# lipku/LiveTalking

Measured on NVIDIA H100. Metric: lip-sync frames/sec (wav2lip256, 256x256, batch 16, mel + U-Net fwd + paste-back), higher is better.
Workload: dtype f16 (fp32 accumulate); mel f64; paste u8

## Files before the change

livetalking_b200/csrc/conv_halo.cu:

```cuda
#include <cuda.h>

#include <atomic>
#include <mutex>
#include <utility>

#include "conv_halo.h"
#include "ltb_internal.h"
#include "ptx_sm90.cuh"

#ifdef LTB_HALO_DIAG
#include <cstdlib>
#define LTB_DIAG(bit) (p.dbg & (bit))
#else
#define LTB_DIAG(bit) 0
#endif

namespace ltb {

constexpr int kHaloP = 10;
constexpr int kHaloThreads = 384;
constexpr int kProducerRegs = 40, kConsumerRegs = 232;
constexpr int kSms = 132;

template <int BN, int NSUB, int NACC, int TAPS, int RC = 0>
struct HaloCfg {
  static constexpr bool HALO = (TAPS != 1);
  static constexpr bool S2 = (TAPS == 10);
  static constexpr int P = S2 ? 9 : (HALO ? kHaloP : 8);
  static constexpr int HR = S2 ? 16 * NSUB + 1 : (HALO ? 16 * NSUB + 2 : 16 * NSUB);
  static constexpr int TG = (TAPS == 9 || TAPS == 10) ? 3 : (TAPS == 16 ? 4 : 1);
  static constexpr int PLANE_BYTES = (HR * P * 128 + 1023) & ~1023;
  static constexpr int A_BYTES_RAW = (S2 ? 4 : 1) * HR * P * 128;
  static constexpr int A_BYTES = S2 ? 4 * PLANE_BYTES : ((A_BYTES_RAW + 1023) & ~1023);
  static constexpr int B_BYTES = TG * BN * 128;
  static constexpr int BUDGET = 223 * 1024;
  static constexpr int A_STAGES_STREAM = S2 ? 2 : ((BN <= 32) ? 4 : (BN <= 64 ? 3 : (NSUB == 1 ? 3 : 2)));
  static constexpr int A_STAGES_RES = ((BUDGET - RC * TG * B_BYTES) / A_BYTES) > 4 ? 4 : ((BUDGET - RC * TG * B_BYTES) / A_BYTES);
  static constexpr int A_STAGES = RC ? A_STAGES_RES : A_STAGES_STREAM;
  static constexpr int B_STAGES_MAX = (BUDGET - A_STAGES * A_BYTES) / B_BYTES;
  static constexpr int B_STAGES = RC ? RC * TG : (B_STAGES_MAX > 8 ? 8 : B_STAGES_MAX);
  static constexpr bool LAG = RC || B_STAGES >= 2 * TG;
  static constexpr int ACOLS = NACC * BN;
  static constexpr int SMEM_BYTES = A_STAGES * A_BYTES + B_STAGES * B_BYTES + 1024;
  static_assert(NSUB * ACOLS <= 256, "register accumulator overflow");
  static_assert(B_STAGES >= 2, "not enough shared memory for the weight ring");
  static_assert(A_STAGES >= 2, "not enough shared memory for the halo ring");
  static_assert(SMEM_BYTES + 3584 <= 227 * 1024, "shared memory overflow (dynamic + static)");
};

struct SubpixelView {
  int stage, view, slot0, brow, nslots;
};
constexpr int subpixel_view(int vy, int vx) { return (vy + 1) * kHaloP + (vx + 1); }
template <int TAPS>
struct SubpixelTable;
template <>
struct SubpixelTable<9> {
  static constexpr int NV = 5;
  static constexpr SubpixelView v[NV] = {{0, 0, 0, 0, 3}, {1, 1, 1, 0, 2}, {1, kHaloP + 1, 2, 2, 1}, {2, 0, 3, 2, 1}, {2, kHaloP, 2, 0, 2}};
};
template <>
struct SubpixelTable<16> {
  static constexpr int NV = 10;
  static constexpr SubpixelView v[NV] = {{0, subpixel_view(0, 0), 0, 0, 4},
                                         {1, subpixel_view(-1, 0), 0, 0, 2},  {1, subpixel_view(0, 1), 1, 2, 2},
                                         {2, subpixel_view(1, 0), 2, 0, 2},   {2, subpixel_view(0, -1), 0, 2, 1}, {2, subpixel_view(0, -1), 3, 3, 1},
                                         {3, subpixel_view(-1, -1), 0, 0, 1}, {3, subpixel_view(-1, 1), 1, 1, 1}, {3, subpixel_view(1, 1), 2, 2, 1},
                                         {3, subpixel_view(1, -1), 3, 3, 1}};
};

template <int BN, int SLOT0, int BROW, int R, size_t... S>
__device__ __forceinline__ void subpixel_slots(float (&acc)[R], uint64_t a, uint32_t b_lo, uint32_t b_hi, std::index_sequence<S...>) {
  (wgmma_ss_at<BN, (SLOT0 + (int)S) * BN>(acc, a, wgmma_lohi(b_lo + (BROW + (uint32_t)S) * BN * 8u, b_hi), 1u), ...);
}

template <int BN, int TAPS, int R, size_t... V>
__device__ __forceinline__ void subpixel_issue(float (&acc)[R], int j, int k, uint32_t a_lo0, uint32_t b_lo0, uint32_t a_hi, uint32_t b_hi,
                                               std::index_sequence<V...>) {
  (
      [&] {
        constexpr SubpixelView g = SubpixelTable<TAPS>::v[V];
        if (j == g.stage)
          subpixel_slots<BN, g.slot0, g.brow>(acc, wgmma_lohi(a_lo0 + g.view * 8u + k * 2u, a_hi), b_lo0 + k * 2u, b_hi,
                                              std::make_index_sequence<g.nslots>{});
      }(),
      ...);
}

__device__ __forceinline__ void quad_transpose(uint32_t (&x)[4], int lane) {
  const bool b2 = lane & 2, b1 = lane & 1;
  uint32_t s0 = __shfl_xor_sync(0xffffffffu, b2 ? x[0] : x[2], 2);
  uint32_t s1 = __shfl_xor_sync(0xffffffffu, b2 ? x[1] : x[3], 2);
  x[0] = b2 ? s0 : x[0];
  x[1] = b2 ? s1 : x[1];
  x[2] = b2 ? x[2] : s0;
  x[3] = b2 ? x[3] : s1;
  s0 = __shfl_xor_sync(0xffffffffu, b1 ? x[0] : x[1], 1);
  s1 = __shfl_xor_sync(0xffffffffu, b1 ? x[2] : x[3], 1);
  x[0] = b1 ? s0 : x[0];
  x[2] = b1 ? s1 : x[2];
  x[1] = b1 ? x[1] : s0;
  x[3] = b1 ? x[3] : s1;
}

constexpr bool halo_res_smem_ok(int BN, int NSUB, int NACC, int TAPS) { return TAPS == 9 && NACC == 1 && BN * NSUB <= 128; }

template <int BN, int NSUB, int NACC, int TAPS, int RC, bool GRP>
__global__ void __launch_bounds__(kHaloThreads, 1) conv_halo_wgmma_kernel(const __grid_constant__ HaloParams p) {
  static_assert(!GRP || TAPS == 1, "grouped weights exist in GEMM mode only");
  using C = HaloCfg<BN, NSUB, NACC, TAPS, RC>;
  extern __shared__ uint8_t smem_raw[];
  __shared__ __align__(8) uint64_t a_full[C::A_STAGES], a_empty[C::A_STAGES];
  __shared__ __align__(8) uint64_t b_full[C::B_STAGES], b_empty[C::B_STAGES];
  __shared__ float head_sw[100];
  constexpr int kGnSmem = (NACC == 1) ? 512 : 1;
  __shared__ float gn_acc[kGnSmem];

  const int tid = threadIdx.x, warp = tid >> 5, lane = tid & 31;
  constexpr bool kHeadOk = (BN == 32 && NACC == 1 && TAPS == 9);
  const bool gn_smem = NACC == 1 && p.gn_stats != nullptr && p.gn_images * p.gn_groups * 2 <= kGnSmem;
  if (gn_smem)
    for (int i = tid; i < p.gn_images * p.gn_groups * 2; i += kHaloThreads) gn_acc[i] = 0.f;
  constexpr bool kHaloMode = C::HALO;
  if (kHeadOk && p.head_out && tid < 99) head_sw[tid] = (tid < 96) ? p.head_w[tid] : p.head_b[tid - 96];
  const uint32_t smem0 = (smem_u32(smem_raw) + 1023u) & ~1023u;
  const uint32_t a_smem = smem0;
  const uint32_t b_smem = smem0 + C::A_STAGES * C::A_BYTES;
  const int chunks = (p.Cin + 63) / 64;

  if (tid == 0) {
    for (int s = 0; s < C::A_STAGES; ++s) {
      mbar_init(smem_u32(&a_full[s]), 1);
      mbar_init(smem_u32(&a_empty[s]), 8);
    }
    for (int s = 0; s < C::B_STAGES; ++s) {
      mbar_init(smem_u32(&b_full[s]), 1);
      mbar_init(smem_u32(&b_empty[s]), 8);
    }
    mbar_fence_init();
    tma_prefetch_desc(&p.tm_in);
    tma_prefetch_desc(&p.tm_w);
  }
  __syncthreads();

  const int tiles_m = kHaloMode ? p.tiles_x * p.tiles_y * p.N : p.tiles_x;

  pdl_launch_dependents();
  if (RC && warp == 8 && lane == 0) {
    mbar_arrive_expect_tx(smem_u32(&b_full[0]), RC * C::TG * C::B_BYTES);
    for (int c = 0; c < RC; ++c)
      for (int j = 0; j < C::TG; ++j)
        tma_load_3d(b_smem + (c * C::TG + j) * C::B_BYTES, &p.tm_w, smem_u32(&b_full[0]), c * 64, 0, j * C::TG);
  }
  pdl_wait();

  if (warp >= 8) {
    setmaxnreg_dec<kProducerRegs>();
    if (warp == 8 && lane == 0) {
      uint32_t ai = 0, bi = 0;
      for (int t = blockIdx.x; t < p.total_tiles; t += gridDim.x) {
        const int nt = t / tiles_m;
        int mt = t - nt * tiles_m;
        int img = 0, y0 = 0, x0 = 0;
        int g_row = 0, g_slot = 0;
        if constexpr (GRP) {
          const int g = mt / p.group_tiles;
          g_row = g * p.group_rows + (mt - g * p.group_tiles) * (128 * NSUB);
          g_slot = p.group_slot[g];
        }
        if (kHaloMode) {
          img = mt / (p.tiles_x * p.tiles_y);
          mt -= img * (p.tiles_x * p.tiles_y);
          const int ty = mt / p.tiles_x, tx = mt - ty * p.tiles_x;
          y0 = ty * (16 * NSUB) + p.halo_y0;
          x0 = tx * 8 + p.halo_x0;
        }
        for (int c = 0; c < chunks; ++c) {
          const uint32_t as = ai % C::A_STAGES;
          mbar_wait(smem_u32(&a_empty[as]), ((ai / C::A_STAGES) & 1u) ^ 1u);
          if (LTB_DIAG(8)) {
            mbar_arrive(smem_u32(&a_full[as]));
          } else {
            mbar_arrive_expect_tx(smem_u32(&a_full[as]), C::A_BYTES_RAW);
            if (C::S2) {
#pragma unroll
              for (int pl = 0; pl < 4; ++pl)
                tma_load_4d(a_smem + as * C::A_BYTES + pl * C::PLANE_BYTES, &p.tm_in, smem_u32(&a_full[as]), c * 64,
                            2 * (x0 + 1) - (pl & 1), 2 * (y0 + 1) - (pl >> 1), img);
            } else if (kHaloMode) tma_load_4d(a_smem + as * C::A_BYTES, &p.tm_in, smem_u32(&a_full[as]), c * 64, x0, y0, img);
            else if constexpr (GRP) tma_load_2d(a_smem + as * C::A_BYTES, &p.tm_in, smem_u32(&a_full[as]), c * 64, g_row);
            else tma_load_2d(a_smem + as * C::A_BYTES, &p.tm_in, smem_u32(&a_full[as]), c * 64, mt * (128 * NSUB));
          }
          ++ai;
          if (RC) continue;
          for (int j = 0; j < C::TG; ++j) {
            const uint32_t bs = bi % C::B_STAGES;
            mbar_wait(smem_u32(&b_empty[bs]), ((bi / C::B_STAGES) & 1u) ^ 1u);
            if (LTB_DIAG(16)) {
              mbar_arrive(smem_u32(&b_full[bs]));
              ++bi;
              continue;
            }
            mbar_arrive_expect_tx(smem_u32(&b_full[bs]), C::B_BYTES);
            if (kHaloMode) tma_load_3d(b_smem + bs * C::B_BYTES, &p.tm_w, smem_u32(&b_full[bs]), c * 64, nt * BN, j * C::TG);
            else if constexpr (GRP) tma_load_3d(b_smem + bs * C::B_BYTES, &p.tm_w, smem_u32(&b_full[bs]), c * 64, nt * BN, g_slot);
            else tma_load_2d(b_smem + bs * C::B_BYTES, &p.tm_w, smem_u32(&b_full[bs]), c * 64, nt * BN);
            ++bi;
          }
        }
      }
    }
  } else {
    setmaxnreg_inc<kConsumerRegs>();
    const int wg = warp >> 2, wq = warp & 3;
    const int cq = 2 * (lane & 3);
    constexpr uint32_t kAHi = wgmma_hi_128b(C::P * 128);
    constexpr uint32_t kBHi = wgmma_hi_128b(1024);
    constexpr uint32_t kRowsPerSub = C::HALO ? 16u * C::P : 128u;
    const uint32_t wg_off = (uint32_t)wg * (C::HALO ? 8u * C::P : 64u) * 8u;
    constexpr bool kResHalo = halo_res_smem_ok(BN, NSUB, NACC, TAPS);
    const int res_row = (8 * wg + 2 * wq + ((lane >> 3) & 1) + 1) * C::P + (lane & 7) + 1;
    const int res_kb = lane >> 4;
    if (RC) mbar_wait(smem_u32(&b_full[0]), 0);
    uint32_t ai = 0, bi = 0;
    for (int t = blockIdx.x; t < p.total_tiles; t += gridDim.x) {
      float acc[NSUB][C::ACOLS / 2];
#pragma unroll
      for (int s = 0; s < NSUB; ++s)
#pragma unroll
        for (int i = 0; i < C::ACOLS / 2; ++i) acc[s][i] = 0.f;
      uint32_t rh[NSUB][2][BN / 8];
      const int n0_res = (t / tiles_m) * BN;
      const int c_res = (kResHalo && p.res_halo) ? n0_res / 64 : chunks;
      const int cb_res = (BN == 32) ? (n0_res & 63) >> 3 : 0;
      uint32_t pend_as = 0, pend_bs = 0;
      bool pend = false;
#pragma unroll 1
      for (int c = 0; c < chunks; ++c) {
        const uint32_t as = ai % C::A_STAGES;
        mbar_wait(smem_u32(&a_full[as]), (ai / C::A_STAGES) & 1u);
        if constexpr (kResHalo) {
          if (c == c_res || (BN == 128 && c == c_res + 1)) {
            const bool hi = BN == 128 && c != c_res;
            const uint32_t rbase = a_smem + as * C::A_BYTES + res_row * 128;
#pragma unroll
            for (int s = 0; s < NSUB; ++s)
#pragma unroll
              for (int i = 0; i < BN / 8; i += 2) {
                if (BN == 128 && (i >= 8) != hi) continue;
                const uint32_t chunk16 = (uint32_t)(((cb_res + i + res_kb) & 7) ^ (res_row & 7));
                ldmatrix_x4(rh[s][0][i], rh[s][1][i], rh[s][0][i + 1], rh[s][1][i + 1], rbase + s * (16 * C::P * 128) + chunk16 * 16);
              }
          }
        }
        const uint32_t a_lo0 = wgmma_lo(a_smem + as * C::A_BYTES) + wg_off;
        const uint32_t bs0 = bi % C::B_STAGES;
#pragma unroll
        for (int j = 0; j < C::TG; ++j) {
          const uint32_t bs = RC ? (uint32_t)(c * C::TG + j) : (bi + j) % C::B_STAGES;
          if (!RC) mbar_wait(smem_u32(&b_full[bs]), ((bi + j) / C::B_STAGES) & 1u);
          const uint32_t b_lo0 = wgmma_lo(b_smem + bs * C::B_BYTES);
          if (!LTB_DIAG(4)) wgmma_fence();
#pragma unroll
          for (int k = 0; k < 4; ++k) {
            if (LTB_DIAG(4)) break;
            if constexpr (NACC == 1) {
#pragma unroll
              for (int tt = 0; tt < C::TG; ++tt) {
                const uint32_t aoff = C::S2 ? (uint32_t)(((j != 1) * 2 + (tt != 1)) * (C::PLANE_BYTES / 16) + ((j == 2) * C::P + (tt == 2)) * 8)
                                            : (kHaloMode ? (uint32_t)(j * C::P + tt) * 8u : 0u);
                const uint64_t bd = wgmma_lohi(b_lo0 + tt * (BN * 8) + k * 2, kBHi);
#pragma unroll
                for (int sub = 0; sub < NSUB; ++sub)
                  Wgmma<BN>::ss(acc[sub], wgmma_lohi(a_lo0 + aoff + sub * kRowsPerSub * 8 + k * 2, kAHi), bd, 1u);
              }
            } else {
              subpixel_issue<BN, TAPS>(acc[0], j, k, a_lo0, b_lo0, kAHi, kBHi, std::make_index_sequence<SubpixelTable<TAPS>::NV>{});
            }
          }
          if constexpr (!C::LAG) {
            wgmma_commit();
            wgmma_wait<0>();
            __syncwarp();
            if (lane == 0) mbar_arrive(smem_u32(&b_empty[bs]));
          }
        }
        if (C::LAG) {
          wgmma_commit();
          wgmma_wait<1>();
          if (pend) {
            __syncwarp();
            if (lane == 0) {
              mbar_arrive(smem_u32(&a_empty[pend_as]));
              if (!RC)
                for (int j = 0; j < C::TG; ++j) mbar_arrive(smem_u32(&b_empty[(pend_bs + j) % C::B_STAGES]));
            }
          }
          pend = true;
          pend_as = as;
          pend_bs = bs0;
        } else {
          __syncwarp();
          if (lane == 0) mbar_arrive(smem_u32(&a_empty[as]));
        }
        ++ai;
        if (!RC) bi += C::TG;
      }
      wgmma_wait<0>();
#pragma unroll
      for (int s = 0; s < NSUB; ++s) wgmma_fence_regs(acc[s]);
      if (C::LAG && pend) {
        __syncwarp();
        if (lane == 0) {
          mbar_arrive(smem_u32(&a_empty[pend_as]));
          if (!RC)
            for (int j = 0; j < C::TG; ++j) mbar_arrive(smem_u32(&b_empty[(pend_bs + j) % C::B_STAGES]));
        }
      }
      if (LTB_DIAG(2)) continue;

      const int nt = t / tiles_m;
      int mt = t - nt * tiles_m;
      int img = 0, ty = 0, tx = 0;
      if (kHaloMode) {
        img = mt / (p.tiles_x * p.tiles_y);
        mt -= img * (p.tiles_x * p.tiles_y);
        ty = mt / p.tiles_x;
        tx = mt - ty * p.tiles_x;
      }
      const int n0 = nt * BN;
      const float* bias = p.bias;
      int g_tile = 0;
      if constexpr (GRP) {
        g_tile = mt / p.group_tiles;
        bias += p.group_slot[g_tile] * p.bias_slot_stride;
      }
      const bool has_res = (p.res != nullptr) && !LTB_DIAG(1);
      const bool res_smem = kResHalo && has_res && p.res_halo;
      const bool res_gmem = has_res && !res_smem;
      const bool head = kHeadOk && p.head_out != nullptr;
      float2 bb[BN / 8];
#pragma unroll
      for (int i = 0; i < BN / 8; ++i) bb[i] = __ldg(reinterpret_cast<const float2*>(bias + n0 + 8 * i + cq));
      const __half2 hmax = __floats2half2_rn(65504.f, 65504.f);
      const __half2 hlo = p.relu ? __floats2half2_rn(0.f, 0.f) : __floats2half2_rn(-65504.f, -65504.f);
      auto add_res = [&](uint32_t v, uint32_t r) {
        const __half2 o = __hmin2(__hmax2(__hadd2(*reinterpret_cast<const __half2*>(&v), *reinterpret_cast<const __half2*>(&r)), hlo), hmax);
        return *reinterpret_cast<const uint32_t*>(&o);
      };
#pragma unroll
      for (int sub = 0; sub < NSUB; ++sub) {
        float gs[BN / 8], gq[BN / 8];
#pragma unroll
        for (int i = 0; i < BN / 8; ++i) gs[i] = gq[i] = 0.f;
#pragma unroll
        for (int sl = 0; sl < NACC; ++sl) {
#pragma unroll
          for (int hh = 0; hh < 2; ++hh) {
            const int r = wq * 16 + (lane >> 2) + 8 * hh;
            size_t opix;
            bool row_ok;
            if (kHaloMode) {
              const int gy = ty * (16 * NSUB) + sub * 16 + wg * 8 + (r >> 3), gx = tx * 8 + (r & 7);
              opix = ((size_t)img * p.OH + gy * p.osy + p.acc_oy[sl]) * p.OW + gx * p.osx + p.acc_ox[sl];
              row_ok = gy < p.GH && gx < p.GW;
            } else if constexpr (GRP) {
              const int lrow = (mt - g_tile * p.group_tiles) * (128 * NSUB) + sub * 128 + wg * 64 + r;
              opix = (size_t)g_tile * p.group_rows + lrow;
              row_ok = lrow < p.group_rows;
            } else {
              opix = (size_t)mt * (128 * NSUB) + sub * 128 + wg * 64 + r;
              row_ok = opix < (size_t)p.M;
            }
            const size_t ocol = n0 + 8 * (lane & 3);
            uint4* optr = reinterpret_cast<uint4*>(p.out + opix * p.OCtot + p.oc_off + ocol);
            const uint4* rptr = res_gmem ? reinterpret_cast<const uint4*>(p.res + opix * p.RCtot + p.rc_off + ocol) : nullptr;
            __half2 oh[BN / 8];
#pragma unroll
            for (int m = 0; m < BN / 32; ++m) {
              uint32_t v[4];
#pragma unroll
              for (int j = 0; j < 4; ++j) {
                const int i = 4 * m + j;
                const float f0 = acc[sub][sl * BN / 2 + 4 * i + 2 * hh] + bb[i].x;
                const float f1 = acc[sub][sl * BN / 2 + 4 * i + 2 * hh + 1] + bb[i].y;
                v[j] = (!has_res && p.relu) ? f32x2_to_f16x2_sat_relu(f0, f1) : f32x2_to_f16x2_sat(f0, f1);
                if constexpr (kResHalo)
                  if (res_smem) v[j] = add_res(v[j], rh[sub][hh][i]);
                oh[i] = *reinterpret_cast<const __half2*>(&v[j]);
              }
              if (!head || res_gmem) {
                quad_transpose(v, lane);
                if (res_gmem) {
                  uint4 r4 = make_uint4(0u, 0u, 0u, 0u);
                  if (row_ok) r4 = __ldcg(rptr + 4 * m);
                  const uint32_t rv[4] = {r4.x, r4.y, r4.z, r4.w};
#pragma unroll
                  for (int j = 0; j < 4; ++j) v[j] = add_res(v[j], rv[j]);
                }
                if (row_ok && !head && !LTB_DIAG(1)) optr[4 * m] = make_uint4(v[0], v[1], v[2], v[3]);
                if (res_gmem && (p.gn_stats || head)) {
                  quad_transpose(v, lane);
#pragma unroll
                  for (int j = 0; j < 4; ++j) oh[4 * m + j] = *reinterpret_cast<const __half2*>(&v[j]);
                }
              }
            }
            if (p.gn_stats && row_ok) {
#pragma unroll
              for (int i = 0; i < BN / 8; ++i) {
                const float2 f = __half22float2(oh[i]);
                gs[i] += f.x + f.y;
                gq[i] += f.x * f.x + f.y * f.y;
              }
            }
            if constexpr (kHeadOk) {
              if (head) {
                uint32_t hv[4][4];
#pragma unroll
                for (int src = 0; src < 4; ++src)
#pragma unroll
                  for (int i = 0; i < 4; ++i)
                    hv[src][i] = __shfl_sync(0xffffffffu, *reinterpret_cast<uint32_t*>(&oh[i]), (lane & ~3) + src);
                if ((lane & 3) == 0 && row_ok) {
                  float ha0 = head_sw[96], ha1 = head_sw[97], ha2 = head_sw[98];
#pragma unroll
                  for (int i = 0; i < 4; ++i)
#pragma unroll
                    for (int src = 0; src < 4; ++src) {
                      const float2 f = __half22float2(*reinterpret_cast<__half2*>(&hv[src][i]));
                      const int cc = 8 * i + 2 * src;
                      ha0 = fmaf(f.x, head_sw[cc], ha0);
                      ha0 = fmaf(f.y, head_sw[cc + 1], ha0);
                      ha1 = fmaf(f.x, head_sw[32 + cc], ha1);
                      ha1 = fmaf(f.y, head_sw[32 + cc + 1], ha1);
                      ha2 = fmaf(f.x, head_sw[64 + cc], ha2);
                      ha2 = fmaf(f.y, head_sw[64 + cc + 1], ha2);
                    }
                  float* o = p.head_out + opix * 3;
                  o[0] = (1.f / (1.f + expf(-ha0))) * 255.f;
                  o[1] = (1.f / (1.f + expf(-ha1))) * 255.f;
                  o[2] = (1.f / (1.f + expf(-ha2))) * 255.f;
                }
              }
            }
          }
        }
        const size_t gn_row0 = (size_t)mt * (128 * NSUB) + sub * 128 + wg * 64 + wq * 16;
        if (p.gn_stats && (kHaloMode || gn_row0 < (size_t)p.M)) {
          int gimg = img;
          if (!kHaloMode) gimg = (int)(gn_row0 / (size_t)p.gn_hw);
          float* sbase = (gn_smem ? gn_acc : p.gn_stats) + (size_t)gimg * p.gn_groups * 2;
#pragma unroll
          for (int i = 0; i < BN / 8; ++i) {
            float a = gs[i], b = gq[i];
#pragma unroll
            for (int o = 4; o < 32; o <<= 1) {
              a += __shfl_xor_sync(0xffffffffu, a, o);
              b += __shfl_xor_sync(0xffffffffu, b, o);
            }
            a += __shfl_xor_sync(0xffffffffu, a, 1);
            b += __shfl_xor_sync(0xffffffffu, b, 1);
            if (p.gn_cpg >= 8) {
              a += __shfl_xor_sync(0xffffffffu, a, 2);
              b += __shfl_xor_sync(0xffffffffu, b, 2);
            }
            if (lane == 0 || (p.gn_cpg == 4 && lane == 2)) {
              const int g = (n0 + 8 * i + cq) / p.gn_cpg;
              atomicAdd(sbase + 2 * g, a);
              atomicAdd(sbase + 2 * g + 1, b);
            }
          }
        }
      }
    }
  }

  __syncthreads();
  if (gn_smem) {
    for (int i = tid; i < p.gn_images * p.gn_groups * 2; i += kHaloThreads) {
      const float v = gn_acc[i];
      if (v != 0.f) atomicAdd(p.gn_stats + i, v);
    }
  }
}

typedef CUresult (*EncodeTiledFn)(CUtensorMap*, CUtensorMapDataType, cuuint32_t, void*, const cuuint64_t*, const cuuint64_t*,
                                  const cuuint32_t*, const cuuint32_t*, CUtensorMapInterleave, CUtensorMapSwizzle,
                                  CUtensorMapL2promotion, CUtensorMapFloatOOBfill);

static EncodeTiledFn get_encode() {
  static EncodeTiledFn fn = nullptr;
  static std::once_flag once;
  std::call_once(once, []() {
    void* p = nullptr;
    cudaDriverEntryPointQueryResult q;
    if (cudaGetDriverEntryPoint("cuTensorMapEncodeTiled", &p, cudaEnableDefault, &q) == cudaSuccess &&
        q == cudaDriverEntryPointSuccess)
      fn = reinterpret_cast<EncodeTiledFn>(p);
  });
  return fn;
}

static bool encode(CUtensorMap* tm, int rank, const void* base, const cuuint64_t* dims, const cuuint64_t* strides_bytes,
                   const cuuint32_t* box, int spatial_stride = 1) {
  EncodeTiledFn fn = get_encode();
  if (!fn) return false;
  cuuint32_t es[5] = {1, (cuuint32_t)spatial_stride, (cuuint32_t)spatial_stride, 1, 1};
  return fn(tm, CU_TENSOR_MAP_DATA_TYPE_FLOAT16, (cuuint32_t)rank, const_cast<void*>(base), dims, strides_bytes, box, es,
            CU_TENSOR_MAP_INTERLEAVE_NONE, CU_TENSOR_MAP_SWIZZLE_128B, CU_TENSOR_MAP_L2_PROMOTION_L2_256B,
            CU_TENSOR_MAP_FLOAT_OOB_FILL_NONE) == CUDA_SUCCESS;
}

static bool is_conv3x3(const ConvParams& p) {
  if (p.nphases != 1 || p.ph[0].ntaps != 9 || p.sy != 1 || p.sx != 1 || p.osy != 1 || p.osx != 1) return false;
  for (int t = 0; t < 9; ++t)
    if (p.ph[0].dy[t] != t / 3 - 1 || p.ph[0].dx[t] != t % 3 - 1) return false;
  return p.IH == p.GH && p.IW == p.GW && p.OH == p.GH && p.OW == p.GW;
}
static bool is_convT(const ConvParams& p) {
  if (p.nphases != 4 || p.osy != 2 || p.osx != 2 || p.sy != 1 || p.sx != 1) return false;
  const int nt[4] = {1, 2, 2, 4};
  for (int i = 0; i < 4; ++i)
    if (p.ph[i].ntaps != nt[i]) return false;
  return p.IH == p.GH && p.IW == p.GW && p.OH == 2 * p.GH && p.OW == 2 * p.GW;
}

static bool is_conv3x3_s2(const ConvParams& p) {
  if (p.nphases != 1 || p.ph[0].ntaps != 9 || p.sy != 2 || p.sx != 2 || p.osy != 1 || p.osx != 1) return false;
  for (int t = 0; t < 9; ++t)
    if (p.ph[0].dy[t] != t / 3 - 1 || p.ph[0].dx[t] != t % 3 - 1) return false;
  return p.IH == 2 * p.GH && p.IW == 2 * p.GW && p.OH == p.GH && p.OW == p.GW;
}

static bool is_upconv(const ConvParams& p) {
  return p.upconv == 1 && p.nphases == 4 && p.osy == 2 && p.osx == 2 && p.sy == 1 && p.sx == 1 && p.IH == p.GH && p.IW == p.GW &&
         p.OH == 2 * p.GH && p.OW == 2 * p.GW;
}

static bool is_gemm(const ConvParams& p) {
  return p.nphases == 1 && p.ph[0].ntaps == 1 && p.ph[0].dy[0] == 0 && p.ph[0].dx[0] == 0 && p.sy == 1 && p.sx == 1 && p.osy == 1 &&
         p.osx == 1 && p.IH == p.GH && p.IW == p.GW && p.OH == p.GH && p.OW == p.GW;
}

static bool pick_cfg(const ConvParams& p, int* BN, int* NSUB, int* NACC);

bool conv_halo_supported(const ConvParams& p) {
  if (p.zbatch > 1) return false;
  if ((p.OCtot % 8) || (p.oc_off % 8) || (reinterpret_cast<uintptr_t>(p.out) % 16)) return false;
  if (p.res && ((p.RCtot % 8) || (p.rc_off % 8) || (reinterpret_cast<uintptr_t>(p.res) % 16))) return false;
  if (p.group_slot && (!is_gemm(p) || (p.w_slot_stride * 2) % 16 != 0)) return false;
  if (is_gemm(p)) {
    return p.Cout % 32 == 0 && p.Cin % 8 == 0 && p.Cin >= 32 && (p.ICtot % 8) == 0 && (p.ic_off % 8) == 0 && (p.Ktot % 8) == 0 &&
           (p.ph[0].koff % 8) == 0 && p.M >= 512 && get_encode() != nullptr;
  }
  if (is_conv3x3_s2(p)) {
    return p.Cout % 32 == 0 && p.Cin >= 64 && (p.ICtot % 8) == 0 && (p.ic_off % 8) == 0 && p.Ktot == 9 * p.Cin && p.GH >= 16 &&
           p.GW >= 8 && get_encode() != nullptr;
  }
  if (is_upconv(p))
    return p.Cout % 64 == 0 && p.Cin >= 16 && (p.ICtot % 8) == 0 && (p.ic_off % 8) == 0 && p.Ktot == 16 * p.Cin && get_encode() != nullptr;
  if (!(is_conv3x3(p) || is_convT(p))) return false;
  if (p.Cout % 32 != 0 || p.Cin < 16) return false;
  if ((p.ICtot % 8) || (p.ic_off % 8) || (p.Ktot != 9 * p.Cin)) return false;
  if (p.GH % 16 != 0 || p.GW % 8 != 0) {
    int BN, NSUB, NACC;
    if (!pick_cfg(p, &BN, &NSUB, &NACC)) return false;
    const long tiles = (long)p.N * ((p.GH + 16 * NSUB - 1) / (16 * NSUB)) * ((p.GW + 7) / 8) * (p.Cout / BN);
    const long waves = (tiles + kSms - 1) / kSms, chunks = (p.Cin + 63) / 64;
    if (waves * chunks > 16) return false;
  }
  return get_encode() != nullptr;
}

static bool pick_cfg(const ConvParams& p, int* BN, int* NSUB, int* NACC) {
  if (is_gemm(p)) {
    *NACC = 1;
    *BN = (p.Cout % 128 == 0) ? 128 : (p.Cout % 64 == 0) ? 64 : 32;
    auto tiles = [&](int bn, int nsub) { return (long)((p.M + 128 * nsub - 1) / (128 * nsub)) * (p.Cout / bn); };
    *NSUB = tiles(*BN, 2) >= kSms ? 2 : 1;
    while (*BN > 32 && tiles(*BN, *NSUB) < kSms - kSms / 8) *BN >>= 1;
    if (*BN == 128) *NSUB = 1;
    return true;
  }
  if (is_upconv(p)) {
    *NACC = 4;
    *NSUB = 1;
    *BN = 64;
    return true;
  }
  if (is_conv3x3_s2(p)) {
    *NACC = 1;
    *NSUB = 1;
    *BN = (p.Cout % 64 == 0) ? 64 : 32;
    return true;
  }
  const bool tr = is_convT(p);
  *NACC = tr ? 4 : 1;
  if (tr) {
    *NSUB = 1;
    *BN = (p.Cout % 64 == 0) ? 64 : 32;
    return true;
  }
  const long ksteps = (p.Cin + 15) / 16;
  double best = 1e30;
  for (int bn : {128, 64, 32}) {
    if (p.Cout % bn) continue;
    for (int nsub : {2, 1}) {
      if (nsub == 2 && (p.GH % 32) != 0) continue;
      const long tiles = (long)p.N * ((p.GH + 16 * nsub - 1) / (16 * nsub)) * ((p.GW + 7) / 8) * (p.Cout / bn);
      const long waves = (tiles + kSms - 1) / kSms;
      const double tile = (double)ksteps * 9 * nsub * (55.0 + 0.2 * bn) + 800.0;
      const double epi = (waves == 1) ? 40.0 * nsub * bn : 0.0;
      const double cost = waves * tile + epi;
      if (cost < best * 0.9) {
        best = cost;
        *BN = bn;
        *NSUB = nsub;
      }
    }
  }
  return best < 1e30;
}

int conv_halo_make_plan(const ConvParams& p, const __half* w_tap_major, HaloPlan* out) {
  if (!conv_halo_supported(p)) return 1;
  HaloParams& h = out->hp;
  std::memset(&h, 0, sizeof(h));
  out->grouped = false;
  int BN, NSUB, NACC;
  if (!pick_cfg(p, &BN, &NSUB, &NACC)) return 1;
  out->BN = BN;
  out->NSUB = NSUB;
  out->NACC = NACC;
  const bool up = is_upconv(p);
  const bool s2 = is_conv3x3_s2(p);
  const bool tr = NACC == 4 && !up;
  const bool gemm = is_gemm(p);
  out->TAPS = gemm ? 1 : (up ? 16 : (s2 ? 10 : 9));
  if (gemm) {
    cuuint64_t dims[2] = {(cuuint64_t)p.Cin, (cuuint64_t)p.M};
    cuuint64_t strides[1] = {(cuuint64_t)p.ICtot * 2};
    cuuint32_t box[2] = {64, (cuuint32_t)(128 * NSUB)};
    if (!encode(&h.tm_in, 2, p.in + p.ic_off, dims, strides, box)) return 2;
    cuuint64_t wdims[3] = {(cuuint64_t)p.Cin, (cuuint64_t)p.Cout, (cuuint64_t)p.slots};
    cuuint64_t wstrides[2] = {(cuuint64_t)p.Ktot * 2, (cuuint64_t)p.w_slot_stride * 2};
    cuuint32_t wbox[3] = {64, (cuuint32_t)BN, 1};
    if (!encode(&h.tm_w, p.group_slot ? 3 : 2, p.w + p.ph[0].koff, wdims, wstrides, wbox)) return 2;
  } else
  {
    cuuint64_t dims[4] = {(cuuint64_t)p.Cin, (cuuint64_t)p.IW, (cuuint64_t)p.IH, (cuuint64_t)p.N};
    cuuint64_t strides[3] = {(cuuint64_t)p.ICtot * 2, (cuuint64_t)p.IW * p.ICtot * 2, (cuuint64_t)p.IH * p.IW * p.ICtot * 2};
    cuuint32_t box[4] = {64, (cuuint32_t)kHaloP, (cuuint32_t)(16 * NSUB + 2), 1};
    if (s2) {
      box[1] = 2 * 9 - 1;
      box[2] = 2 * (16 * NSUB + 1) - 1;
    }
    if (!encode(&h.tm_in, 4, p.in + p.ic_off, dims, strides, box, s2 ? 2 : 1)) return 2;
  }
  if (up) {
    cuuint64_t dims[3] = {(cuuint64_t)p.Cin, (cuuint64_t)p.Cout, 16};
    cuuint64_t strides[2] = {(cuuint64_t)p.Cin * 2, (cuuint64_t)p.Cout * p.Cin * 2};
    cuuint32_t box[3] = {64, (cuuint32_t)BN, 4};
    if (!encode(&h.tm_w, 3, w_tap_major, dims, strides, box)) return 2;
  } else if (!gemm) {
    cuuint64_t dims[3] = {(cuuint64_t)p.Cin, (cuuint64_t)p.Cout, 9};
    cuuint64_t strides[2] = {(cuuint64_t)p.Cin * 2, (cuuint64_t)p.Cout * p.Cin * 2};
    cuuint32_t box[3] = {64, (cuuint32_t)BN, 3};
    if (!encode(&h.tm_w, 3, w_tap_major, dims, strides, box)) return 2;
  }
  h.out = p.out;
  h.res = p.res;
  h.bias = p.bias;
  h.N = p.N;
  h.M = p.M;
  h.Cin = p.Cin;
  h.gn_stats = nullptr;
#ifdef LTB_HALO_DIAG
  if (const char* e = std::getenv("LTB_HALO_DIAG")) h.dbg = std::atoi(e);
#endif
  h.OCtot = p.OCtot;
  h.oc_off = p.oc_off;
  h.RCtot = p.RCtot;
  h.rc_off = p.rc_off;
  h.OH = p.OH;
  h.OW = p.OW;
  h.GH = p.GH;
  h.GW = p.GW;
  h.osy = p.osy;
  h.osx = p.osx;
  h.relu = p.relu;
  h.res_halo = halo_res_smem_ok(BN, NSUB, NACC, out->TAPS) && p.res != nullptr && p.res == p.in && p.Cin == p.Cout &&
               p.rc_off == p.ic_off && p.RCtot == p.ICtot;
  h.halo_y0 = tr ? 0 : -1;
  h.halo_x0 = tr ? 0 : -1;
  if (up || tr) {
    const int slot_phase[4] = {0, 1, 3, 2};
    for (int sl = 0; sl < 4; ++sl) {
// ... 153 lines not shown
```

livetalking_b200/csrc/ptx_sm90.cuh:

```cuda
#pragma once
#include <cuda_fp16.h>
#include <cstdint>
#include <cstdio>

namespace ltb {

__device__ __forceinline__ uint32_t smem_u32(const void* p) {
  return static_cast<uint32_t>(__cvta_generic_to_shared(p));
}

__device__ __forceinline__ void mbar_init(uint32_t bar, uint32_t count) {
  asm volatile("mbarrier.init.shared::cta.b64 [%0], %1;" ::"r"(bar), "r"(count) : "memory");
}
__device__ __forceinline__ void mbar_fence_init() {
  asm volatile("fence.mbarrier_init.release.cluster;" ::: "memory");
}
__device__ __forceinline__ void mbar_arrive(uint32_t bar) {
  asm volatile("mbarrier.arrive.shared::cta.b64 _, [%0];" ::"r"(bar) : "memory");
}
__device__ __forceinline__ void mbar_arrive_expect_tx(uint32_t bar, uint32_t bytes) {
  asm volatile("mbarrier.arrive.expect_tx.shared::cta.b64 _, [%0], %1;" ::"r"(bar), "r"(bytes) : "memory");
}
__device__ __forceinline__ bool mbar_try_wait(uint32_t bar, uint32_t parity) {
  uint32_t ok;
  asm volatile(
      "{\n\t.reg .pred p;\n\t"
      "mbarrier.try_wait.parity.shared::cta.b64 p, [%1], %2;\n\t"
      "selp.u32 %0, 1, 0, p;\n\t}"
      : "=r"(ok)
      : "r"(bar), "r"(parity)
      : "memory");
  return ok != 0;
}
__device__ __forceinline__ void mbar_wait(uint32_t bar, uint32_t parity) {
  if (mbar_try_wait(bar, parity)) return;
  const long long t0 = clock64();
  while (!mbar_try_wait(bar, parity)) {
    if (clock64() - t0 > 8000000000LL) __trap();
  }
}

__device__ __forceinline__ void fence_proxy_async_smem() {
  asm volatile("fence.proxy.async.shared::cta;" ::: "memory");
}

__device__ __forceinline__ void cp_async16(uint32_t dst, const void* src, uint32_t src_bytes) {
  asm volatile("cp.async.cg.shared.global [%0], [%1], 16, %2;" ::"r"(dst), "l"(src), "r"(src_bytes) : "memory");
}
__device__ __forceinline__ void cp_async_commit() { asm volatile("cp.async.commit_group;" ::: "memory"); }
template <int N>
__device__ __forceinline__ void cp_async_wait() {
  asm volatile("cp.async.wait_group %0;" ::"n"(N) : "memory");
}

__device__ __forceinline__ void tma_prefetch_desc(const void* tmap) {
  asm volatile("prefetch.tensormap [%0];" ::"l"(tmap) : "memory");
}
__device__ __forceinline__ void tma_load_2d(uint32_t dst, const void* tmap, uint32_t bar, int c0, int c1) {
  asm volatile(
      "cp.async.bulk.tensor.2d.shared::cluster.global.mbarrier::complete_tx::bytes [%0], [%1, {%3, %4}], [%2];" ::"r"(dst),
      "l"(tmap), "r"(bar), "r"(c0), "r"(c1)
      : "memory");
}
__device__ __forceinline__ void tma_load_3d(uint32_t dst, const void* tmap, uint32_t bar, int c0, int c1, int c2) {
  asm volatile(
      "cp.async.bulk.tensor.3d.shared::cluster.global.mbarrier::complete_tx::bytes [%0], [%1, {%3, %4, %5}], [%2];" ::"r"(dst),
      "l"(tmap), "r"(bar), "r"(c0), "r"(c1), "r"(c2)
      : "memory");
}
__device__ __forceinline__ void tma_load_4d(uint32_t dst, const void* tmap, uint32_t bar, int c0, int c1, int c2, int c3) {
  asm volatile(
      "cp.async.bulk.tensor.4d.shared::cluster.global.mbarrier::complete_tx::bytes [%0], [%1, {%3, %4, %5, %6}], [%2];" ::"r"(
          dst),
      "l"(tmap), "r"(bar), "r"(c0), "r"(c1), "r"(c2), "r"(c3)
      : "memory");
}
__device__ __forceinline__ void tma_load_5d(uint32_t dst, const void* tmap, uint32_t bar, int c0, int c1, int c2, int c3,
                                            int c4) {
  asm volatile(
      "cp.async.bulk.tensor.5d.shared::cluster.global.mbarrier::complete_tx::bytes [%0], [%1, {%3, %4, %5, %6, %7}], [%2];" ::
          "r"(dst),
      "l"(tmap), "r"(bar), "r"(c0), "r"(c1), "r"(c2), "r"(c3), "r"(c4)
      : "memory");
}

__device__ __forceinline__ void ldmatrix_x4(uint32_t& r0, uint32_t& r1, uint32_t& r2, uint32_t& r3, uint32_t saddr) {
  asm volatile("ldmatrix.sync.aligned.m8n8.x4.shared.b16 {%0, %1, %2, %3}, [%4];"
               : "=r"(r0), "=r"(r1), "=r"(r2), "=r"(r3)
               : "r"(saddr)
               : "memory");
}

__device__ __forceinline__ uint64_t wgmma_desc(uint32_t saddr, uint32_t lbo_bytes, uint32_t sbo_bytes, uint32_t layout) {
  uint64_t d = 0;
  d |= (uint64_t)((saddr & 0x3FFFF) >> 4);
  d |= (uint64_t)((lbo_bytes >> 4) & 0x3FFF) << 16;
  d |= (uint64_t)((sbo_bytes >> 4) & 0x3FFF) << 32;
  d |= (uint64_t)(layout & 3) << 62;
  return d;
}
__host__ __device__ constexpr uint32_t wgmma_hi_128b(uint32_t sbo_bytes) { return (sbo_bytes >> 4) | (1u << 30); }
__device__ __forceinline__ uint32_t wgmma_lo(uint32_t saddr) { return ((saddr & 0x3FFFFu) >> 4) | (1u << 16); }
__device__ __forceinline__ uint64_t wgmma_lohi(uint32_t lo, uint32_t hi) { return ((uint64_t)hi << 32) | lo; }

__device__ __forceinline__ void wgmma_fence() { asm volatile("wgmma.fence.sync.aligned;" ::: "memory"); }
__device__ __forceinline__ void wgmma_commit() { asm volatile("wgmma.commit_group.sync.aligned;" ::: "memory"); }
template <int N>
__device__ __forceinline__ void wgmma_wait() {
  asm volatile("wgmma.wait_group.sync.aligned %0;" ::"n"(N) : "memory");
}
template <int R>
__device__ __forceinline__ void wgmma_fence_regs(float (&d)[R]) {
#pragma unroll
  for (int i = 0; i < R; ++i) asm volatile("" : "+f"(d[i])::"memory");
}

template <int N>
struct Wgmma;
#define LTB_D1(i) "+f"(d[i])
#define LTB_D2(i) LTB_D1(i), LTB_D1(i + 1)
#define LTB_D4(i) LTB_D2(i), LTB_D2(i + 2)
#define LTB_D8(i) LTB_D4(i), LTB_D4(i + 4)
#define LTB_D16(i) LTB_D8(i), LTB_D8(i + 8)
#define LTB_D32(i) LTB_D16(i), LTB_D16(i + 16)
#define LTB_D64(i) LTB_D32(i), LTB_D32(i + 32)
#define LTB_D128(i) LTB_D64(i), LTB_D64(i + 64)
#define LTB_WG_HEAD(P) "{\n.reg .pred p;\nsetp.ne.b32 p, %" P ", 0;\nwgmma.mma_async.sync.aligned.m64n"
#define LTB_WG_SS(N, REGS, A, B, P) LTB_WG_HEAD(P) N "k16.f32.f16.f16 " REGS ", %" A ", %" B ", p, 1, 1, 0, 0;\n}\n"
#define LTB_WG_RS(N, REGS, A, B, P) \
  LTB_WG_HEAD(P) N "k16.f32.f16.f16 " REGS ", {%" A "}, %" B ", p, 1, 1, 0;\n}\n"

template <>
struct Wgmma<16> {
#define LTB_R "{%0,%1,%2,%3,%4,%5,%6,%7}"
  __device__ __forceinline__ static void ss(float (&d)[8], uint64_t a, uint64_t b, uint32_t acc) {
    asm volatile(LTB_WG_SS("16", LTB_R, "8", "9", "10") : LTB_D8(0) : "l"(a), "l"(b), "r"(acc));
  }
  __device__ __forceinline__ static void rs(float (&d)[8], const uint32_t (&a)[4], uint64_t b, uint32_t acc) {
    asm volatile(LTB_WG_RS("16", LTB_R, "8,%9,%10,%11", "12", "13") : LTB_D8(0)
                 : "r"(a[0]), "r"(a[1]), "r"(a[2]), "r"(a[3]), "l"(b), "r"(acc));
  }
#undef LTB_R
};

template <>
struct Wgmma<32> {
#define LTB_R "{%0,%1,%2,%3,%4,%5,%6,%7,%8,%9,%10,%11,%12,%13,%14,%15}"
  __device__ __forceinline__ static void ss(float (&d)[16], uint64_t a, uint64_t b, uint32_t acc) {
    asm volatile(LTB_WG_SS("32", LTB_R, "16", "17", "18") : LTB_D16(0) : "l"(a), "l"(b), "r"(acc));
  }
  __device__ __forceinline__ static void rs(float (&d)[16], const uint32_t (&a)[4], uint64_t b, uint32_t acc) {
    asm volatile(LTB_WG_RS("32", LTB_R, "16,%17,%18,%19", "20", "21") : LTB_D16(0)
                 : "r"(a[0]), "r"(a[1]), "r"(a[2]), "r"(a[3]), "l"(b), "r"(acc));
  }
#undef LTB_R
};

template <>
struct Wgmma<48> {
#define LTB_R "{%0,%1,%2,%3,%4,%5,%6,%7,%8,%9,%10,%11,%12,%13,%14,%15,%16,%17,%18,%19,%20,%21,%22,%23}"
  __device__ __forceinline__ static void rs(float (&d)[24], const uint32_t (&a)[4], uint64_t b, uint32_t acc) {
    asm volatile(LTB_WG_RS("48", LTB_R, "24,%25,%26,%27", "28", "29") : LTB_D16(0), LTB_D8(16)
                 : "r"(a[0]), "r"(a[1]), "r"(a[2]), "r"(a[3]), "l"(b), "r"(acc));
  }
#undef LTB_R
};

template <>
struct Wgmma<64> {
#define LTB_R "{%0,%1,%2,%3,%4,%5,%6,%7,%8,%9,%10,%11,%12,%13,%14,%15,%16,%17,%18,%19,%20,%21,%22,%23,%24,%25,%26,%27,%28,%29,%30,%31}"
  __device__ __forceinline__ static void ss(float (&d)[32], uint64_t a, uint64_t b, uint32_t acc) {
    asm volatile(LTB_WG_SS("64", LTB_R, "32", "33", "34") : LTB_D32(0) : "l"(a), "l"(b), "r"(acc));
  }
  __device__ __forceinline__ static void rs(float (&d)[32], const uint32_t (&a)[4], uint64_t b, uint32_t acc) {
    asm volatile(LTB_WG_RS("64", LTB_R, "32,%33,%34,%35", "36", "37") : LTB_D32(0)
                 : "r"(a[0]), "r"(a[1]), "r"(a[2]), "r"(a[3]), "l"(b), "r"(acc));
  }
#undef LTB_R
};

template <>
struct Wgmma<80> {
#define LTB_R "{%0,%1,%2,%3,%4,%5,%6,%7,%8,%9,%10,%11,%12,%13,%14,%15,%16,%17,%18,%19,%20,%21,%22,%23,%24,%25,%26,%27,%28,%29,%30,%31,%32,%33,%34,%35,%36,%37,%38,%39}"
  __device__ __forceinline__ static void rs(float (&d)[40], const uint32_t (&a)[4], uint64_t b, uint32_t acc) {
    asm volatile(LTB_WG_RS("80", LTB_R, "40,%41,%42,%43", "44", "45") : LTB_D32(0), LTB_D8(32)
                 : "r"(a[0]), "r"(a[1]), "r"(a[2]), "r"(a[3]), "l"(b), "r"(acc));
  }
#undef LTB_R
};

template <>
struct Wgmma<96> {
#define LTB_R "{%0,%1,%2,%3,%4,%5,%6,%7,%8,%9,%10,%11,%12,%13,%14,%15,%16,%17,%18,%19,%20,%21,%22,%23,%24,%25,%26,%27,%28,%29,%30,%31,%32,%33,%34,%35,%36,%37,%38,%39,%40,%41,%42,%43,%44,%45,%46,%47}"
  __device__ __forceinline__ static void ss(float (&d)[48], uint64_t a, uint64_t b, uint32_t acc) {
    asm volatile(LTB_WG_SS("96", LTB_R, "48", "49", "50") : LTB_D32(0), LTB_D16(32) : "l"(a), "l"(b), "r"(acc));
  }
  __device__ __forceinline__ static void rs(float (&d)[48], const uint32_t (&a)[4], uint64_t b, uint32_t acc) {
    asm volatile(LTB_WG_RS("96", LTB_R, "48,%49,%50,%51", "52", "53") : LTB_D32(0), LTB_D16(32)
                 : "r"(a[0]), "r"(a[1]), "r"(a[2]), "r"(a[3]), "l"(b), "r"(acc));
  }
#undef LTB_R
};

template <>
struct Wgmma<112> {
#define LTB_R "{%0,%1,%2,%3,%4,%5,%6,%7,%8,%9,%10,%11,%12,%13,%14,%15,%16,%17,%18,%19,%20,%21,%22,%23,%24,%25,%26,%27,%28,%29,%30,%31,%32,%33,%34,%35,%36,%37,%38,%39,%40,%41,%42,%43,%44,%45,%46,%47,%48,%49,%50,%51,%52,%53,%54,%55}"
  __device__ __forceinline__ static void rs(float (&d)[56], const uint32_t (&a)[4], uint64_t b, uint32_t acc) {
    asm volatile(LTB_WG_RS("112", LTB_R, "56,%57,%58,%59", "60", "61") : LTB_D32(0), LTB_D16(32), LTB_D8(48)
                 : "r"(a[0]), "r"(a[1]), "r"(a[2]), "r"(a[3]), "l"(b), "r"(acc));
  }
#undef LTB_R
};

template <>
struct Wgmma<128> {
#define LTB_R "{%0,%1,%2,%3,%4,%5,%6,%7,%8,%9,%10,%11,%12,%13,%14,%15,%16,%17,%18,%19,%20,%21,%22,%23,%24,%25,%26,%27,%28,%29,%30,%31,%32,%33,%34,%35,%36,%37,%38,%39,%40,%41,%42,%43,%44,%45,%46,%47,%48,%49,%50,%51,%52,%53,%54,%55,%56,%57,%58,%59,%60,%61,%62,%63}"
  __device__ __forceinline__ static void ss(float (&d)[64], uint64_t a, uint64_t b, uint32_t acc) {
    asm volatile(LTB_WG_SS("128", LTB_R, "64", "65", "66") : LTB_D64(0) : "l"(a), "l"(b), "r"(acc));
  }
  __device__ __forceinline__ static void rs(float (&d)[64], const uint32_t (&a)[4], uint64_t b, uint32_t acc) {
    asm volatile(LTB_WG_RS("128", LTB_R, "64,%65,%66,%67", "68", "69") : LTB_D64(0)
                 : "r"(a[0]), "r"(a[1]), "r"(a[2]), "r"(a[3]), "l"(b), "r"(acc));
  }
#undef LTB_R
};

template <>
struct Wgmma<144> {
#define LTB_R "{%0,%1,%2,%3,%4,%5,%6,%7,%8,%9,%10,%11,%12,%13,%14,%15,%16,%17,%18,%19,%20,%21,%22,%23,%24,%25,%26,%27,%28,%29,%30,%31,%32,%33,%34,%35,%36,%37,%38,%39,%40,%41,%42,%43,%44,%45,%46,%47,%48,%49,%50,%51,%52,%53,%54,%55,%56,%57,%58,%59,%60,%61,%62,%63,%64,%65,%66,%67,%68,%69,%70,%71}"
  __device__ __forceinline__ static void rs(float (&d)[72], const uint32_t (&a)[4], uint64_t b, uint32_t acc) {
    asm volatile(LTB_WG_RS("144", LTB_R, "72,%73,%74,%75", "76", "77") : LTB_D64(0), LTB_D8(64)
                 : "r"(a[0]), "r"(a[1]), "r"(a[2]), "r"(a[3]), "l"(b), "r"(acc));
  }
#undef LTB_R
};

template <>
struct Wgmma<160> {
#define LTB_R "{%0,%1,%2,%3,%4,%5,%6,%7,%8,%9,%10,%11,%12,%13,%14,%15,%16,%17,%18,%19,%20,%21,%22,%23,%24,%25,%26,%27,%28,%29,%30,%31,%32,%33,%34,%35,%36,%37,%38,%39,%40,%41,%42,%43,%44,%45,%46,%47,%48,%49,%50,%51,%52,%53,%54,%55,%56,%57,%58,%59,%60,%61,%62,%63,%64,%65,%66,%67,%68,%69,%70,%71,%72,%73,%74,%75,%76,%77,%78,%79}"
  __device__ __forceinline__ static void rs(float (&d)[80], const uint32_t (&a)[4], uint64_t b, uint32_t acc) {
    asm volatile(LTB_WG_RS("160", LTB_R, "80,%81,%82,%83", "84", "85") : LTB_D64(0), LTB_D16(64)
                 : "r"(a[0]), "r"(a[1]), "r"(a[2]), "r"(a[3]), "l"(b), "r"(acc));
  }
#undef LTB_R
};

template <>
struct Wgmma<192> {
#define LTB_R "{%0,%1,%2,%3,%4,%5,%6,%7,%8,%9,%10,%11,%12,%13,%14,%15,%16,%17,%18,%19,%20,%21,%22,%23,%24,%25,%26,%27,%28,%29,%30,%31,%32,%33,%34,%35,%36,%37,%38,%39,%40,%41,%42,%43,%44,%45,%46,%47,%48,%49,%50,%51,%52,%53,%54,%55,%56,%57,%58,%59,%60,%61,%62,%63,%64,%65,%66,%67,%68,%69,%70,%71,%72,%73,%74,%75,%76,%77,%78,%79,%80,%81,%82,%83,%84,%85,%86,%87,%88,%89,%90,%91,%92,%93,%94,%95}"
  __device__ __forceinline__ static void ss(float (&d)[96], uint64_t a, uint64_t b, uint32_t acc) {
    asm volatile(LTB_WG_SS("192", LTB_R, "96", "97", "98") : LTB_D64(0), LTB_D32(64) : "l"(a), "l"(b), "r"(acc));
  }
#undef LTB_R
};

template <>
struct Wgmma<256> {
#define LTB_R "{%0,%1,%2,%3,%4,%5,%6,%7,%8,%9,%10,%11,%12,%13,%14,%15,%16,%17,%18,%19,%20,%21,%22,%23,%24,%25,%26,%27,%28,%29,%30,%31,%32,%33,%34,%35,%36,%37,%38,%39,%40,%41,%42,%43,%44,%45,%46,%47,%48,%49,%50,%51,%52,%53,%54,%55,%56,%57,%58,%59,%60,%61,%62,%63,%64,%65,%66,%67,%68,%69,%70,%71,%72,%73,%74,%75,%76,%77,%78,%79,%80,%81,%82,%83,%84,%85,%86,%87,%88,%89,%90,%91,%92,%93,%94,%95,%96,%97,%98,%99,%100,%101,%102,%103,%104,%105,%106,%107,%108,%109,%110,%111,%112,%113,%114,%115,%116,%117,%118,%119,%120,%121,%122,%123,%124,%125,%126,%127}"
  __device__ __forceinline__ static void ss(float (&d)[128], uint64_t a, uint64_t b, uint32_t acc) {
    asm volatile(LTB_WG_SS("256", LTB_R, "128", "129", "130") : LTB_D128(0) : "l"(a), "l"(b), "r"(acc));
  }
#undef LTB_R
};

template <int N, int C0, int R>
__device__ __forceinline__ void wgmma_ss_at(float (&d)[R], uint64_t a, uint64_t b, uint32_t acc) {
  static_assert(C0 % 8 == 0 && C0 / 2 + N / 2 <= R, "accumulator slice out of range");
  Wgmma<N>::ss(*reinterpret_cast<float(*)[N / 2]>(&d[C0 / 2]), a, b, acc);
}

__device__ __forceinline__ uint32_t f32x2_to_f16x2_sat(float lo, float hi) {
  uint32_t r;
  asm("cvt.rn.satfinite.f16x2.f32 %0, %1, %2;" : "=r"(r) : "f"(hi), "f"(lo));
  return r;
}
__device__ __forceinline__ uint32_t f32x2_to_f16x2_sat_relu(float lo, float hi) {
  uint32_t r;
  asm("cvt.rn.relu.satfinite.f16x2.f32 %0, %1, %2;" : "=r"(r) : "f"(hi), "f"(lo));
  return r;
}

__device__ __forceinline__ void pdl_wait() { asm volatile("griddepcontrol.wait;" ::: "memory"); }
__device__ __forceinline__ void pdl_launch_dependents() { asm volatile("griddepcontrol.launch_dependents;" ::: "memory"); }

template <uint32_t N>
__device__ __forceinline__ void setmaxnreg_inc() {
  asm volatile("setmaxnreg.inc.sync.aligned.u32 %0;" ::"n"(N));
}
template <uint32_t N>
__device__ __forceinline__ void setmaxnreg_dec() {
  asm volatile("setmaxnreg.dec.sync.aligned.u32 %0;" ::"n"(N));
}

__device__ __forceinline__ bool elect_one() {
  uint32_t pred;
  asm volatile(
      "{\n\t.reg .pred p;\n\t"
      "elect.sync _|p, 0xffffffff;\n\t"
      "selp.u32 %0, 1, 0, p;\n\t}"
      : "=r"(pred));
  return pred != 0;
}

}
```

Baseline: 6435.

## Prefetch residual tiles during the mainloop for BN128 3x3 halo convs

For one specific conv configuration (BN=128, NSUB=2, 3x3 taps, streaming weights), the consumer warps now issue cp.async loads of the first sub-tile's residual into a dedicated shared-memory buffer before the K loop. They also load the second sub-tile's residual into registers before waiting on the final wgmma. This hides global residual-load latency in the epilogue behind the MMA mainloop. The cost is shared memory carved from the weight ring, which may cut B stages, plus extra live registers in the consumer.

```diff
diff --git a/livetalking_b200/csrc/conv_halo.cu b/livetalking_b200/csrc/conv_halo.cu
--- a/livetalking_b200/csrc/conv_halo.cu
+++ b/livetalking_b200/csrc/conv_halo.cu
@@ -37,11 +37,13 @@
   static constexpr int A_STAGES_STREAM = S2 ? 2 : ((BN <= 32) ? 4 : (BN <= 64 ? 3 : (NSUB == 1 ? 3 : 2)));
   static constexpr int A_STAGES_RES = ((BUDGET - RC * TG * B_BYTES) / A_BYTES) > 4 ? 4 : ((BUDGET - RC * TG * B_BYTES) / A_BYTES);
   static constexpr int A_STAGES = RC ? A_STAGES_RES : A_STAGES_STREAM;
-  static constexpr int B_STAGES_MAX = (BUDGET - A_STAGES * A_BYTES) / B_BYTES;
+  static constexpr bool RES_PREFETCH = (BN == 128 && NSUB == 2 && NACC == 1 && TAPS == 9 && RC == 0);
+  static constexpr int RES_BYTES = RES_PREFETCH ? 128 * BN * 2 : 0;
+  static constexpr int B_STAGES_MAX = (BUDGET - A_STAGES * A_BYTES - RES_BYTES) / B_BYTES;
   static constexpr int B_STAGES = RC ? RC * TG : (B_STAGES_MAX > 8 ? 8 : B_STAGES_MAX);
   static constexpr bool LAG = RC || B_STAGES >= 2 * TG;
   static constexpr int ACOLS = NACC * BN;
-  static constexpr int SMEM_BYTES = A_STAGES * A_BYTES + B_STAGES * B_BYTES + 1024;
+  static constexpr int SMEM_BYTES = A_STAGES * A_BYTES + B_STAGES * B_BYTES + RES_BYTES + 1024;
   static_assert(NSUB * ACOLS <= 256, "register accumulator overflow");
   static_assert(B_STAGES >= 2, "not enough shared memory for the weight ring");
   static_assert(A_STAGES >= 2, "not enough shared memory for the halo ring");
@@ -221,9 +223,43 @@
     constexpr bool kResHalo = halo_res_smem_ok(BN, NSUB, NACC, TAPS);
     const int res_row = (8 * wg + 2 * wq + ((lane >> 3) & 1) + 1) * C::P + (lane & 7) + 1;
     const int res_kb = lane >> 4;
+    auto halo_pix = [&](int img, int ty, int tx, int sub, int sl, int r, bool& ok) -> size_t {
+      const int gy = ty * (16 * NSUB) + sub * 16 + wg * 8 + (r >> 3), gx = tx * 8 + (r & 7);
+      ok = gy < p.GH && gx < p.GW;
+      return ((size_t)img * p.OH + gy * p.osy + p.acc_oy[sl]) * p.OW + gx * p.osx + p.acc_ox[sl];
+    };
+    const uint32_t res_buf = b_smem + C::B_STAGES * C::B_BYTES;
     if (RC) mbar_wait(smem_u32(&b_full[0]), 0);
     uint32_t ai = 0, bi = 0;
     for (int t = blockIdx.x; t < p.total_tiles; t += gridDim.x) {
+      const int nt = t / tiles_m;
+      int mt = t - nt * tiles_m;
+      int img = 0, ty = 0, tx = 0;
+      if (kHaloMode) {
+        img = mt / (p.tiles_x * p.tiles_y);
+        mt -= img * (p.tiles_x * p.tiles_y);
+        ty = mt / p.tiles_x;
+        tx = mt - ty * p.tiles_x;
+      }
+      const int n0 = nt * BN;
+      const bool res_pf = C::RES_PREFETCH && p.res != nullptr && !LTB_DIAG(1);
+      auto res_src = [&](int sub, int r, bool& ok) {
+        const size_t px = halo_pix(img, ty, tx, sub, 0, r, ok);
+        return reinterpret_cast<const uint4*>(p.res + (ok ? px : 0) * p.RCtot + p.rc_off + n0 + 8 * (lane & 3));
+      };
+      if constexpr (C::RES_PREFETCH) {
+        if (res_pf) {
+#pragma unroll
+          for (int hh = 0; hh < 2; ++hh) {
+            bool ok;
+            const uint4* src = res_src(0, wq * 16 + (lane >> 2) + 8 * hh, ok);
+#pragma unroll
+            for (int m = 0; m < BN / 32; ++m) cp_async16(res_buf + ((hh * (BN / 32) + m) * 256 + tid) * 16, src + 4 * m, ok ? 16u : 0u);
+          }
+          cp_async_commit();
+        }
+      }
+      uint4 rpf[2][BN / 32];
       float acc[NSUB][C::ACOLS / 2];
 #pragma unroll
       for (int s = 0; s < NSUB; ++s)
@@ -306,7 +342,19 @@
         ++ai;
         if (!RC) bi += C::TG;
       }
+      if constexpr (C::RES_PREFETCH) {
+        if (res_pf) {
+#pragma unroll
+          for (int hh = 0; hh < 2; ++hh) {
+            bool ok;
+            const uint4* src = res_src(1, wq * 16 + (lane >> 2) + 8 * hh, ok);
+#pragma unroll
+            for (int m = 0; m < BN / 32; ++m) rpf[hh][m] = ok ? __ldcg(src + 4 * m) : make_uint4(0u, 0u, 0u, 0u);
+          }
+        }
+      }
       wgmma_wait<0>();
+      if (C::RES_PREFETCH && res_pf) cp_async_wait<0>();
 #pragma unroll
       for (int s = 0; s < NSUB; ++s) wgmma_fence_regs(acc[s]);
       if (C::LAG && pend) {
@@ -319,16 +367,6 @@
       }
       if (LTB_DIAG(2)) continue;
 
-      const int nt = t / tiles_m;
-      int mt = t - nt * tiles_m;
-      int img = 0, ty = 0, tx = 0;
-      if (kHaloMode) {
-        img = mt / (p.tiles_x * p.tiles_y);
-        mt -= img * (p.tiles_x * p.tiles_y);
-        ty = mt / p.tiles_x;
-        tx = mt - ty * p.tiles_x;
-      }
-      const int n0 = nt * BN;
       const float* bias = p.bias;
       int g_tile = 0;
       if constexpr (GRP) {
@@ -361,9 +399,7 @@
             size_t opix;
             bool row_ok;
             if (kHaloMode) {
-              const int gy = ty * (16 * NSUB) + sub * 16 + wg * 8 + (r >> 3), gx = tx * 8 + (r & 7);
-              opix = ((size_t)img * p.OH + gy * p.osy + p.acc_oy[sl]) * p.OW + gx * p.osx + p.acc_ox[sl];
-              row_ok = gy < p.GH && gx < p.GW;
+              opix = halo_pix(img, ty, tx, sub, sl, r, row_ok);
             } else if constexpr (GRP) {
               const int lrow = (mt - g_tile * p.group_tiles) * (128 * NSUB) + sub * 128 + wg * 64 + r;
               opix = (size_t)g_tile * p.group_rows + lrow;
@@ -393,7 +429,8 @@
                 quad_transpose(v, lane);
                 if (res_gmem) {
                   uint4 r4 = make_uint4(0u, 0u, 0u, 0u);
-                  if (row_ok) r4 = __ldcg(rptr + 4 * m);
+                  if constexpr (C::RES_PREFETCH) r4 = sub == 0 ? lds128(res_buf + ((hh * (BN / 32) + m) * 256 + tid) * 16) : rpf[hh][m];
+                  else if (row_ok) r4 = __ldcg(rptr + 4 * m);
                   const uint32_t rv[4] = {r4.x, r4.y, r4.z, r4.w};
 #pragma unroll
                   for (int j = 0; j < 4; ++j) v[j] = add_res(v[j], rv[j]);
diff --git a/livetalking_b200/csrc/ptx_sm90.cuh b/livetalking_b200/csrc/ptx_sm90.cuh
--- a/livetalking_b200/csrc/ptx_sm90.cuh
+++ b/livetalking_b200/csrc/ptx_sm90.cuh
@@ -51,6 +51,11 @@
 template <int N>
 __device__ __forceinline__ void cp_async_wait() {
   asm volatile("cp.async.wait_group %0;" ::"n"(N) : "memory");
+}
+__device__ __forceinline__ uint4 lds128(uint32_t addr) {
+  uint4 v;
+  asm volatile("ld.shared.v4.u32 {%0, %1, %2, %3}, [%4];" : "=r"(v.x), "=r"(v.y), "=r"(v.z), "=r"(v.w) : "r"(addr) : "memory");
+  return v;
 }
 
 __device__ __forceinline__ void tma_prefetch_desc(const void* tmap) {
```

New measurement: 6693, median of 6. 1.04x the previous value.
